# StephenTaf/Modern-Search-Engines-Project

Measured on AMD Instinct MI355X. Metric: queries/sec, two-stage retrieval top-100 (BM25 top-1000 + dense full scan + rerank/fuse), higher is better.
Workload: dtype f32 (exact f32 cosines of every returned document; candidates filtered by one pass of f16 products with a measured margin; batches <= 64 queries: f16x2-split products, |err| <= 8e-6) (dense cosine) / f64 (BM25, fuse)

## Files before the change

### modern-search-engines-project_amd/csrc/msr_gemm.hip

```cpp
#include <type_traits>

#include "msr_common.h"
#include "msr_internal.h"
#include "msr_frag.h"
#include "msr_gemm_dev.h"

namespace {


__global__ __launch_bounds__(256) void unit_bf16_rows_kernel(const float* __restrict__ src, const float* __restrict__ inv_norm,
                                                              int64_t n_rows, int64_t n_pad, bf16x8* __restrict__ dst,
                                                              uint32_t* __restrict__ err_max) {
    const int lane = threadIdx.x & 63;
    const int64_t wave = (int64_t)blockIdx.x * 4 + (threadIdx.x >> 6), n_waves = (int64_t)gridDim.x * 4;
    float worst = 0.f;
    for (int64_t r = wave; r < n_pad; r += n_waves) {
        float ss = 0.f;
#pragma unroll
        for (int h = 0; h < 2; ++h) {
            const int c = lane + 64 * h;
            if (c >= MSR_DIM / 8) continue;
            bf16x8 v;
            if (r < n_rows) {
                const float sc = inv_norm ? inv_norm[r] : 1.0f;
// ... 89 lines not shown
        }
    }
}

__global__ __launch_bounds__(1024) void gemm_kth_kernel(const float* __restrict__ tmax, int n, int stride, int nq, int k,
                                                         const float* __restrict__ margin, float* __restrict__ thr,
                                                         int32_t* __restrict__ flag, float short_val, float margin_scale,
                                                         int raise) {
    __shared__ uint32_t hist[2048];
    __shared__ uint32_t wsum[16];
    __shared__ uint32_t s_bin, s_kk, s_hit;
    const int q = blockIdx.x, t = threadIdx.x, lane = t & 63, wave = t >> 6;
    if (q >= nq) {
        if (t == 0 && !raise) { thr[q] = short_val; if (flag) flag[q] = 0; }
        return;
    }
    const float* row = tmax + (size_t)q * stride;
    uint32_t prefix = 0, mask = 0, kk = (uint32_t)k;
    bool short_row = false;
#pragma unroll 1
    for (int pass = 0; pass < 3; ++pass) {
        const int shift = pass == 0 ? 21 : pass == 1 ? 10 : 0;
        const uint32_t nb = pass == 2 ? 1024u : 2048u;
        hist[t] = 0; hist[t + 1024] = 0;
        if (t == 0) s_hit = 0;
        __syncthreads();
        for (int i = t; i < n; i += 1024) {
            const float x = row[i];
            if (!msr_valid(x)) continue;
            const uint32_t key = msr_ord32(x);
            if ((key & mask) == prefix) atomicAdd(&hist[(key >> shift) & (nb - 1)], 1u);
        }
        __syncthreads();
        const uint32_t h0 = 2 * t < (int)nb ? hist[2 * t] : 0u, h1 = 2 * t + 1 < (int)nb ? hist[2 * t + 1] : 0u;
        const uint32_t c2 = h0 + h1;
        uint32_t inc = c2;
#pragma unroll
        for (int o = 1; o < 64; o <<= 1) {
            const uint32_t v = __shfl_down(inc, o);
            if (lane + o < 64) inc += v;
        }
        if (lane == 0) wsum[wave] = inc;
        __syncthreads();
        uint32_t above = inc - c2;
        for (int w2 = wave + 1; w2 < 16; ++w2) above += wsum[w2];
        if (above < kk && kk <= above + c2) {
            if (above + h1 >= kk) { s_bin = 2 * t + 1; s_kk = kk - above; }
            else { s_bin = 2 * t; s_kk = kk - above - h1; }
            s_hit = 1;
        }
        __syncthreads();
        if (!s_hit) { short_row = true; break; }
        prefix |= s_bin << shift;
        mask |= (nb - 1) << shift;
        kk = s_kk;
        __syncthreads();
    }
    if (t == 0) {
        const float v = short_row ? short_val : msr_unord32(prefix) - (margin ? margin_scale * margin[q] : 0.0f);
        if (raise) {
            if (!short_row && v > thr[q]) thr[q] = v;
        } else {
            thr[q] = v;
            if (flag) flag[q] = short_row ? 1 : 0;
        }
    }
}


__global__ __launch_bounds__(256) void gemm_bucket_kernel(const int4* __restrict__ wgbuf, int wg_cap,
                                                           const int32_t* __restrict__ wg_count,
                                                           const float* __restrict__ thr2, int2* __restrict__ pairs,
                                                           int pair_cap, int32_t* __restrict__ pair_n) {
    const int wg = blockIdx.y;
    int n = wg_count[wg];
    if (n > wg_cap) n = wg_cap;
    for (int i = blockIdx.x * 256 + threadIdx.x; i < n; i += gridDim.x * 256) {
        const int4 e = wgbuf[(size_t)wg * wg_cap + i];
        if (__int_as_float(e.z) >= thr2[e.y]) {
            const int pos = atomicAdd(&pair_n[e.y], 1);
            if (pos < pair_cap) pairs[(size_t)e.y * pair_cap + pos] = make_int2(e.x, e.z);
        }
    }
}

constexpr int GM_PAIR_CAP = 4096;
static_assert(GM_PAIR_CAP <= (1 << 13), "cand_first_len packs first and len into 13 bits each");
__global__ __launch_bounds__(1024) void gemm_cand_kernel(int2* __restrict__ pairs, int32_t* __restrict__ pair_n,
                                                          const int32_t* __restrict__ chunk_doc, int64_t n_rows,
                                                          const int32_t* __restrict__ wg_count, int n_wg, int wg_cap,
                                                          const int32_t* __restrict__ flag, int k,
                                                          const float* __restrict__ margin,
                                                          int32_t* __restrict__ cand_doc, int32_t* __restrict__ cand_first_len,
                                                          int32_t* __restrict__ cand_n) {
    __shared__ uint64_t key[GM_PAIR_CAP];
    __shared__ uint32_t pay[GM_PAIR_CAP];
    __shared__ int s_heads, s_over;
    const int q = blockIdx.x, t = threadIdx.x;
    const int raw = pair_n[q];
    int over = raw > GM_PAIR_CAP || (flag && flag[q]);
    for (int i = t; i < n_wg; i += 1024) over |= wg_count[i] > wg_cap;
    if (t == 0) s_heads = 0;
    s_over = 0;
    __syncthreads();
    if (over) s_over = 1;
    __syncthreads();
    if (s_over) {
        if (t == 0) { cand_n[q] = MSR_SEL_CAP + 1; pair_n[q] = 0; }
        return;
    }
    int P = 64;
    while (P < raw) P <<= 1;
    auto sort_desc = [&]() {
        for (int kk = 2; kk <= P; kk <<= 1)
            for (int j = kk >> 1; j > 0; j >>= 1) {
                for (int idx = t; idx < (P >> 1); idx += 1024) {
                    const int i = ((idx & ~(j - 1)) << 1) | (idx & (j - 1));
                    const int p = i | j;
                    const bool desc = (i & kk) == 0;
                    const uint64_t x = key[i], y = key[p];
                    if (desc ? x < y : x > y) {
                        key[i] = y; key[p] = x;
                        const uint32_t v = pay[i]; pay[i] = pay[p]; pay[p] = v;
                    }
                }
                __syncthreads();
            }
    };
    for (int i = t; i < P; i += 1024) {
        uint64_t kk = 0;
        uint32_t row = 0;
        if (i < raw) {
            const int2 e = pairs[(size_t)q * GM_PAIR_CAP + i];
            if (e.x >= 0 && e.x < n_rows) {
                kk = ((uint64_t)(uint32_t)(chunk_doc[e.x] + 1) << 32) | msr_ord32(__int_as_float(e.y));
                row = (uint32_t)e.x;
            }
        }
        key[i] = kk; pay[i] = row;
    }
    __syncthreads();
    sort_desc();
    uint64_t mine[GM_PAIR_CAP / 1024];
    uint32_t mine_run[GM_PAIR_CAP / 1024];
#pragma unroll
    for (int u = 0; u < GM_PAIR_CAP / 1024; ++u) {
        const int i = t + u * 1024;
        uint64_t kk = 0;
        uint32_t run = 0;
        if (i < P && key[i] != 0) {
            pairs[(size_t)q * GM_PAIR_CAP + i].x = (int32_t)pay[i];
            const uint32_t d = (uint32_t)(key[i] >> 32);
            if (i == 0 || (uint32_t)(key[i - 1] >> 32) != d) {
                kk = ((uint64_t)(uint32_t)key[i] << 32) | (uint32_t)~(uint32_t)(d - 1);
                int len = 1;
                while (i + len < P && (uint32_t)(key[i + len] >> 32) == d) ++len;
                run = (uint32_t)i | ((uint32_t)len << 13);
            }
        }
        mine[u] = kk; mine_run[u] = run;
    }
    __syncthreads();
#pragma unroll
    for (int u = 0; u < GM_PAIR_CAP / 1024; ++u) {
        const int i = t + u * 1024;
        if (i < P) {
            key[i] = mine[u]; pay[i] = mine_run[u];
            if (mine[u]) atomicAdd(&s_heads, 1);
        }
    }
    __syncthreads();
    sort_desc();
    const int heads = s_heads;
    const float tk = heads >= k ? msr_unord32((uint32_t)(key[k - 1] >> 32)) : -__builtin_inff();
    const float cut = tk - margin[q];
    __shared__ int s_keep;
    if (t == 0) s_keep = 0;
    __syncthreads();
    for (int i = t; i < heads; i += 1024)
        if (msr_unord32((uint32_t)(key[i] >> 32)) >= cut) {
            atomicAdd(&s_keep, 1);
            if (i < MSR_SEL_CAP) {
                cand_doc[(size_t)q * MSR_SEL_CAP + i] = (int32_t)~(uint32_t)key[i];
                cand_first_len[(size_t)q * MSR_SEL_CAP + i] = (int32_t)pay[i];
            }
        }
    __syncthreads();
    if (t == 0) { cand_n[q] = s_keep; pair_n[q] = 0; }
}

int g_gemm_dbg = 0;

}

hipError_t msr_unit_bf16_rows(const float* src, const float* inv_norm, int64_t n_rows, int64_t n_pad, void* dst,
                              uint32_t* err_max, hipStream_t stream) {
    if (n_pad <= 0) return hipSuccess;
    hipError_t err = err_max ? hipMemsetAsync(err_max, 0, 4, stream) : hipSuccess;
    if (err != hipSuccess) return err;
    unit_bf16_rows_kernel<<<8192, 256, 0, stream>>>(src, inv_norm, n_rows, n_pad, (bf16x8*)dst, err_max);
    return hipGetLastError();
}

hipError_t msr_batch_margin(const float* qn, int nq, const uint32_t* err_max, float* margin, hipStream_t stream) {
    if (nq <= 0) return hipSuccess;
    batch_margin_kernel<<<(nq + 3) / 4, 256, 0, stream>>>(qn, nq, err_max, margin);
    return hipGetLastError();
}

int msr_gemm_pair_cap() { return GM_PAIR_CAP; }

hipError_t msr_gemm_tmax(const float* tmax_t, int n_j, int parts, int nq_pad, float* out, int out_stride, hipStream_t stream) {
    if (n_j <= 0 || nq_pad <= 0) return hipSuccess;
    if (parts <= 0 || nq_pad % 128 != 0) return hipErrorInvalidValue;
    const dim3 grid((n_j + 31) / 32, nq_pad / 128);
    if (parts == 8) gemm_tmax_kernel<8><<<grid, 256, 0, stream>>>(tmax_t, n_j, parts, nq_pad, out, out_stride);
    else if (parts == 1) gemm_tmax_kernel<1><<<grid, 256, 0, stream>>>(tmax_t, n_j, parts, nq_pad, out, out_stride);
    else gemm_tmax_kernel<0><<<grid, 256, 0, stream>>>(tmax_t, n_j, parts, nq_pad, out, out_stride);
    return hipGetLastError();
}
hipError_t msr_gemm_kth(const float* tmax, int n, int stride, int nq, int nq_pad, int k, const float* margin, float* thr,
                        int32_t* flag, hipStream_t stream, float short_val, float margin_scale, bool raise) {
    if (nq_pad <= 0) return hipSuccess;
    gemm_kth_kernel<<<nq_pad, 1024, 0, stream>>>(tmax, n, stride, nq, k, margin, thr, raise ? nullptr : flag, short_val, margin_scale,
                                                 raise ? 1 : 0);
    return hipGetLastError();
}
hipError_t msr_gemm_bucket(const void* wvbuf, int wv_cap, const int32_t* wv_count, int n_waves, const float* thr2,
                           void* pairs, int32_t* pair_n, hipStream_t stream) {
    gemm_bucket_kernel<<<dim3(2, (unsigned)n_waves), 256, 0, stream>>>((const int4*)wvbuf, wv_cap, wv_count, thr2, (int2*)pairs,
                                                                      GM_PAIR_CAP, pair_n);
    return hipGetLastError();
}
void msr_gemm_set_dbg(int v) { g_gemm_dbg = v; }

hipError_t msr_gemm_candidates(const GemmIndex& g, const DenseIndex& ix, const float* qn, int nq, int k, const float* margin,
                               int32_t* cand_doc, int32_t* cand_first_len, int32_t* cand_n, hipEvent_t* ev, hipStream_t stream) {
    const int nq_pad = (nq + 255) / 256 * 256;
    const int nt = nq_pad / 256;
    if (nq <= 0 || nq_pad > g.max_queries || k < 1 || g.n_tiles < 2 * k) return hipErrorInvalidValue;
    const int grid = g.n_cus / 8 * 8;
    if (grid < 8 || grid / 8 < nt) return hipErrorInvalidValue;
    hipError_t err;
    int ss = g.n_tiles / (8 * k);
    ss = ss < 1 ? 1 : (ss > 16 ? 16 : ss);
#ifdef MSR_DIAG
    if (g_gemm_dbg & 256) ss = 1;
#endif
    const int n_s = (g.n_tiles - ss / 2 + ss - 1) / ss;
    {
        if ((err = msr_stream256_bf16_qimage(qn, nq, nt, g.qmat, stream)) != hipSuccess) return err;
        StreamArgs a{};
        a.E = (const char*)g.emb_n; a.inv_pad = nullptr; a.qimg = (const char*)g.qmat; a.tile_row = g.tile_row;
        a.n_rows = ix.n_chunks; a.tmax_t = g.tmax_t; a.nt = nt; a.q_base = 0; a.append = 0;
        a.t_first = ss / 2; a.t_stride = ss; a.t_count = n_s;
        if (ev && (err = hipEventRecord(ev[0], stream)) != hipSuccess) return err;
        if ((err = msr_stream256_bf16_launch(false, a, grid, stream)) != hipSuccess) return err;
        if (ev && (err = hipEventRecord(ev[1], stream)) != hipSuccess) return err;
        if ((err = msr_gemm_tmax(g.tmax_t, n_s, 1, nq_pad, (float*)g.tmax, g.tmax_stride, stream)) != hipSuccess) return err;
        gemm_kth_kernel<<<nq_pad, 1024, 0, stream>>>((const float*)g.tmax, n_s, g.tmax_stride, nq, k, margin, g.thr, g.flag, __builtin_inff(), 1.0f, 0);
        a.t_first = 0; a.t_stride = 1; a.t_count = g.n_tiles;
        a.thr = g.thr; a.wvbuf = g.wgbuf; a.wv_cap = g.wv_cap; a.wv_count = g.wv_count;
        if (ev && (err = hipEventRecord(ev[2], stream)) != hipSuccess) return err;
        if ((err = msr_stream256_bf16_launch(true, a, grid, stream)) != hipSuccess) return err;
        if (ev && (err = hipEventRecord(ev[3], stream)) != hipSuccess) return err;
        if ((err = msr_gemm_tmax(g.tmax_t, g.n_tiles, 1, nq_pad, (float*)g.tmax, g.tmax_stride, stream)) != hipSuccess) return err;
        gemm_kth_kernel<<<nq_pad, 1024, 0, stream>>>((const float*)g.tmax, g.n_tiles, g.tmax_stride, nq, k, margin, g.thr2, nullptr, __builtin_inff(), 1.0f, 0);
    }
    gemm_bucket_kernel<<<dim3(2, (unsigned)grid * 8), 256, 0, stream>>>((const int4*)g.wgbuf, g.wv_cap, g.wv_count, g.thr2,
                                                                       (int2*)g.pairs, GM_PAIR_CAP, g.pair_n);
    gemm_cand_kernel<<<nq, 1024, 0, stream>>>((int2*)g.pairs, g.pair_n, ix.chunk_doc, ix.n_chunks, g.wv_count, grid * 8, g.wv_cap,
                                              g.flag, k, margin, cand_doc, cand_first_len, cand_n);
    return hipGetLastError();
}
```

### modern-search-engines-project_amd/csrc/msr_gemm_f32.hip

```cpp
#include <cmath>
#include <type_traits>

#include "msr_common.h"
#include "msr_internal.h"
#include "msr_frag.h"
#include "msr_gemm_dev.h"

namespace {

constexpr int GF_THREADS = 512;
constexpr int GF_KT = MSR_DIM / 32;
constexpr int GF_ROWB = MSR_DIM * 4;
constexpr int GF_PAIR_CAP = 4096;

typedef StreamArgs GemmF32Args;

__device__ __forceinline__ const char* uniform_ptr(const char* p) {
    const uint64_t u = (uint64_t)p;
    const uint32_t lo = __builtin_amdgcn_readfirstlane((uint32_t)u), hi = __builtin_amdgcn_readfirstlane((uint32_t)(u >> 32));
    return (const char*)(((uint64_t)hi << 32) | lo);
}

constexpr int GS_NB = 8;
constexpr int GS_STEP = 8192;
// ... 248 lines not shown
template <int OFF, bool NT = false>
__device__ __forceinline__ void gload16s(f32x4& r, uint32_t voff, uint64_t sbase) {
    if (NT) asm volatile("global_load_dwordx4 %0, %1, %2 offset:%3 nt" : "=v"(r) : "v"(voff), "s"(sbase), "n"(OFF) : "memory");
    else asm volatile("global_load_dwordx4 %0, %1, %2 offset:%3" : "=v"(r) : "v"(voff), "s"(sbase), "n"(OFF) : "memory");
}
__device__ __forceinline__ f16x8 take16(const f32x4& r) {
    f32x4 o;
    asm volatile("v_mov_b32 %0, %1" : "=v"(o[0]) : "v"(r[0]));
    asm volatile("v_mov_b32 %0, %1" : "=v"(o[1]) : "v"(r[1]));
    asm volatile("v_mov_b32 %0, %1" : "=v"(o[2]) : "v"(r[2]));
    asm volatile("v_mov_b32 %0, %1" : "=v"(o[3]) : "v"(r[3]));
    return __builtin_bit_cast(f16x8, o);
}
__device__ __forceinline__ uint32_t fresh_lane() {
    uint32_t l;
    asm volatile("v_mbcnt_lo_u32_b32 %0, -1, 0\n\tv_mbcnt_hi_u32_b32 %0, -1, %0" : "=v"(l));
    return l;
}
typedef __attribute__((address_space(3))) char lds_char;
template <int OFF>
__device__ __forceinline__ void lds_read16(f16x8& r, uint32_t addr) {
    asm volatile("ds_read_b128 %0, %1 offset:%2" : "=v"(r) : "v"(addr), "n"(OFF) : "memory");
}
__device__ __forceinline__ uint64_t uniform_u64(uint64_t u) {
    const uint32_t lo = __builtin_amdgcn_readfirstlane((uint32_t)u), hi = __builtin_amdgcn_readfirstlane((uint32_t)(u >> 32));
    return ((uint64_t)hi << 32) | lo;
}

template <bool EMIT, bool BF16, bool TILED = false, bool NTL = false, bool F16I = false>
__global__ __launch_bounds__(G2_THREADS) void gemm_stream256_kernel(GemmF32Args a) {
    static_assert(!F16I || (BF16 && !TILED && !NTL), "the f16 image takes the 16-bit image's data path");
    static_assert(!(BF16 && TILED), "the fragment-order copy exists for the f32 rows only");
    extern __shared__ __attribute__((aligned(16))) char smem[];
    constexpr int ROWB = BF16 ? MSR_DIM * 2 : GF_ROWB;
    constexpr int KPS = BF16 ? 2 : 1;
    constexpr int RSLOTS = G2_NB / KPS;
    constexpr int NMI = 2, NNI = 16;
    constexpr int WROWS = 16 * NMI;
    static_assert((G2_THREADS / 64) * WROWS == MSR_STREAM256_TILE_ROWS, "the fragment-order copy is padded for this many rows per tile visit");
    const int tid = threadIdx.x, lane = tid & 63;
    const int w = __builtin_amdgcn_readfirstlane(tid >> 6);
    const int wr = w, wc = 0;
    const int li16 = lane & 15, lg = lane >> 4;
    const int nt = a.nt;
    int G = (int)gridDim.x, gid = (int)blockIdx.x, grp = 0;
    bool active = true;
    if (nt > 1) {
        const int per_x = (int)gridDim.x >> 3, xcd = (int)blockIdx.x & 7, li = (int)blockIdx.x >> 3;
        const int gpx = per_x / nt, mg = li / nt;
        grp = li - mg * nt;
        G = __builtin_amdgcn_readfirstlane(8 * gpx);
        gid = __builtin_amdgcn_readfirstlane(xcd * gpx + mg);
        grp = __builtin_amdgcn_readfirstlane(grp);
        active = mg < gpx;
    }
    const int nq_pad = nt * 256;
    int wave_cnt = EMIT && a.append ? __builtin_amdgcn_readfirstlane(a.wv_count[blockIdx.x * 8 + w]) : 0;
    int4* wvbuf = EMIT ? (int4*)a.wvbuf + ((size_t)blockIdx.x * 8 + w) * a.wv_cap : nullptr;
    if (!active || gid >= a.t_count) {
        if (EMIT && lane == 0) a.wv_count[blockIdx.x * 8 + w] = wave_cnt;
        return;
    }
    const int n_mine = __builtin_amdgcn_readfirstlane((a.t_count - gid + G - 1) / G);
    const char* qimg = a.qimg + (size_t)grp * (GF_KT * G2_STEP);
    const int q_base = a.q_base + grp * 256;
    float* thr_lds = (float*)(smem + 2 * G2_BLK);
    if (EMIT && tid < 256) thr_lds[tid] = a.thr[grp * 256 + tid];
    constexpr bool THR_REGS = EMIT && !BF16;
    uint32_t thr_h[THR_REGS ? NNI / 2 : 1];
    if (THR_REGS) {
        auto down_h = [](float x) -> uint32_t {
            _Float16 h = (_Float16)x;
            uint16_t b = __builtin_bit_cast(uint16_t, h);
            if ((float)h > x) b = (b & 0x8000u) ? (uint16_t)(b + 1) : (b == 0 ? (uint16_t)0x8001u : (uint16_t)(b - 1));
            return b;
        };
#pragma unroll
        for (int j = 0; j < NNI / 2; ++j) {
            const float lo = a.thr[grp * 256 + (2 * j) * 16 + li16], hi = a.thr[grp * 256 + (2 * j + 1) * 16 + li16];
            thr_h[j] = down_h(lo) | (down_h(hi) << 16);
        }
    }
    constexpr bool JOIN = BF16;
    uint32_t* tmx = (uint32_t*)(smem + G2_TMX);
    if (JOIN) tmx[tid] = 0u;
    auto flush_tmax = [&](int tile_j, int par) {
        const int ln = (int)fresh_lane();
        if (ln < 32) {
            uint32_t* slot = tmx + par * 256 + w * 32 + ln;
            a.tmax_t[(size_t)tile_j * nq_pad + grp * 256 + w * 32 + ln] = ord_val(*slot);
            *slot = 0u;
        }
    };
    float* inv_lds = (float*)(smem + 2 * G2_BLK + 1024) + w * 64;
    auto stage_b = [&](int blk, int pb) {
        const char* base = uniform_ptr(qimg + (size_t)blk * G2_BLK + (size_t)w * 8192);
#pragma unroll
        for (int i = 0; i < 8; ++i)
            __builtin_amdgcn_global_load_lds((glb_void*)(base + (uint32_t)(i * 1024 + lane * 16)),
                                             (lds_void*)(smem + pb * G2_BLK + w * 8192 + i * 1024), 16, 0, 0);
    };
    f32x4 acc[NMI][NNI];
#pragma unroll
    for (int mi = 0; mi < NMI; ++mi)
#pragma unroll
        for (int ni = 0; ni < NNI; ++ni) acc[mi][ni] = (f32x4){0.f, 0.f, 0.f, 0.f};

    auto tile_of = [&](int j) { return a.t_first + j * a.t_stride; };
    auto tile_base = [&](int row0) { return uniform_u64((uint64_t)a.E + (uint64_t)row0 * ROWB); };
    constexpr int NV = (BF16 || TILED) ? 1 : NMI;
    auto row_off = [&](int row0, int mi) -> uint32_t {
        if (TILED) return (uint32_t)(lane * 16);
        if (BF16) return (uint32_t)((WROWS * wr + li16) * ROWB + lg * 32);
        int64_t r = (int64_t)row0 + WROWS * wr + 16 * mi + li16;
        if (r > a.n_rows - 1) r = a.n_rows - 1;
        return (uint32_t)((r - row0) * ROWB + lg * 32);
    };
    int jt = gid;
    int row0 = a.tile_row[tile_of(jt)], row_end = a.tile_row[tile_of(jt) + 1];
    int jn = jt + G < a.t_count ? jt + G : jt;
    int row0n = a.tile_row[tile_of(jn)];
    uint64_t bp = tile_base(TILED ? a.tile_trow[tile_of(jt)] : row0), bn = tile_base(TILED ? a.tile_trow[tile_of(jn)] : row0n);
    uint32_t vp[NV], vn[NV];
#pragma unroll
    for (int mi = 0; mi < NV; ++mi) { vp[mi] = row_off(row0, mi); vn[mi] = row_off(row0n, mi); }

    static_assert(NMI == 2, "the wait counts below assume 4 row loads per ring slot");
    f32x4 ring[RSLOTS][NMI][2];
    auto load_rows = [&](auto slot_c, uint64_t sb, const uint32_t* v, auto off_c) {
        constexpr int slot = decltype(slot_c)::value, off = decltype(off_c)::value;
#pragma unroll
        for (int mi = 0; mi < NMI; ++mi) {
            if (TILED) {
                const uint64_t b = sb + (uint64_t)((2 * wr + mi) * ((GF_KT / KPS) * 2048) + slot * 2048);
                gload16s<0, NTL>(ring[slot][mi][0], v[0], b);
                gload16s<1024, NTL>(ring[slot][mi][1], v[0], b);
            } else {
                const uint64_t b = BF16 ? sb + (uint64_t)(mi * 16 * ROWB) : sb;
                gload16s<off, NTL>(ring[slot][mi][0], v[BF16 ? 0 : mi], b);
                gload16s<off + 16, NTL>(ring[slot][mi][1], v[BF16 ? 0 : mi], b);
            }
        }
    };
    auto pin_rows = [&](auto slot_c) {
        constexpr int slot = decltype(slot_c)::value;
        pin4(ring[slot][0][0], ring[slot][0][1], ring[slot][1][0], ring[slot][1][1]);
    };
    constexpr int NKB = GF_KT / G2_NB;
    constexpr int BLKB = TILED ? RSLOTS * 2048 : RSLOTS * 128;
    stage_b(0, 0);
#pragma unroll
    for (int s = 0; s < RSLOTS; ++s)
#pragma unroll
        for (int mi = 0; mi < NMI; ++mi) ring[s][mi][0] = ring[s][mi][1] = (f32x4){0.f, 0.f, 0.f, 0.f};
    load_rows(std::integral_constant<int, 0>{}, bp, vp, std::integral_constant<int, 0>{});
    load_rows(std::integral_constant<int, 1>{}, bp, vp, std::integral_constant<int, 128>{});
    if (!BF16) {
        load_rows(std::integral_constant<int, RSLOTS - 2>{}, bp, vp, std::integral_constant<int, 256>{});
        load_rows(std::integral_constant<int, RSLOTS - 1>{}, bp, vp, std::integral_constant<int, 384>{});
    }
    wait_vm0();
    pin_rows(std::integral_constant<int, 0>{}); pin_rows(std::integral_constant<int, 1>{});
    pin_rows(std::integral_constant<int, RSLOTS - 2>{}); pin_rows(std::integral_constant<int, RSLOTS - 1>{});
    wg_barrier();
    int pb = 0;

// ... 101 lines not shown
        for (int kb = 0; kb < NKB; ++kb) {
            const bool last = kb == NKB - 1;
            const int kn = last ? 0 : kb + 1;
#ifdef MSR_DIAG
            if (!(a.dbg & 524288))
#endif
            stage_b(kn, pb ^ 1);
            step(std::integral_constant<int, 0>{}, kn, last);
            step(std::integral_constant<int, 1>{}, kn, last);
            step(std::integral_constant<int, 2>{}, kn, last);
            step(std::integral_constant<int, 3>{}, kn, last);
            if (BF16) asm volatile("s_waitcnt vmcnt(8)" ::: "memory");
            else asm volatile("s_waitcnt vmcnt(16)" ::: "memory");
#ifdef MSR_DIAG
            if (!(a.dbg & 131072))
#endif
            wg_barrier();
            pb ^= 1;
            if (JOIN && kb == 0 && it > 0) flush_tmax(jt_prev, (it - 1) & 1);
        }
        const int ln_e = (int)fresh_lane();
        const int lg_e = ln_e >> 4;
        f32x4 inv4[NMI];
        if (!BF16 || F16I) {
            if (F16I) asm volatile("s_waitcnt vmcnt(8)" ::: "memory");
            else asm volatile("s_waitcnt vmcnt(12)" ::: "memory");
#pragma unroll
            for (int mi = 0; mi < NMI; ++mi) inv4[mi] = *(const f32x4*)(inv_lds + mi * 16 + 4 * lg_e);
        }
        const int n_valid = row_end - row0;
        const int col_e = wc * 128 + (ln_e & 15);
        float thr_nx = (EMIT && !THR_REGS) ? thr_lds[col_e] : 0.f;
#ifdef MSR_DIAG
        if (a.dbg & 65536) {
#pragma unroll
            for (int ni = 0; ni < NNI; ++ni)
#pragma unroll
                for (int mi = 0; mi < NMI; ++mi) acc[mi][ni] = (f32x4){0.f, 0.f, 0.f, 0.f};
        } else
#endif
#pragma unroll
        for (int ni = 0; ni < NNI; ++ni) {
            f32x4 v[NMI];
            float cmax = NEG_INF;
            const float thr_cur = thr_nx;
            if (EMIT && !THR_REGS && ni + 1 < NNI) thr_nx = thr_lds[(ni + 1) * 16 + col_e];
#pragma unroll
            for (int mi = 0; mi < NMI; ++mi) {
                const int blk = wr * WROWS + mi * 16;
                if (BF16 && !F16I) v[mi] = acc[mi][ni];
                else v[mi] = acc[mi][ni] * inv4[mi];
                if (blk + 16 > n_valid) {
#pragma unroll
                    for (int rr = 0; rr < 4; ++rr)
                        if (blk + 4 * lg_e + rr >= n_valid) v[mi][rr] = NEG_INF;
                }
                cmax = max2_raw(cmax, max3_raw(max2_raw(v[mi][0], v[mi][1]), v[mi][2], v[mi][3]));
                acc[mi][ni] = (f32x4){0.f, 0.f, 0.f, 0.f};
            }
            if (EMIT) {
                float thr;
                if (THR_REGS) thr = (float)__builtin_bit_cast(_Float16, (uint16_t)(ni & 1 ? thr_h[ni >> 1] >> 16 : thr_h[ni >> 1] & 0xffffu));
                else thr = thr_cur;
                if (__ballot(cmax >= thr) != 0) {
                    const int q = q_base + ni * 16 + col_e;
#pragma unroll
                    for (int mi = 0; mi < NMI; ++mi) {
                        const int rb = wr * WROWS + mi * 16 + 4 * lg_e;
#pragma unroll
                        for (int rr = 0; rr < 4; ++rr) {
                            const float x = v[mi][rr];
                            const bool hit = x >= thr;
                            const unsigned long long hm = __ballot(hit);
                            if (hm != 0) {
                                const int pos = wave_cnt + (int)__builtin_amdgcn_mbcnt_hi((uint32_t)(hm >> 32), __builtin_amdgcn_mbcnt_lo((uint32_t)hm, 0u));
                                if (hit && pos < a.wv_cap)
                                    wvbuf[pos] = make_int4(row0 + rb + rr, q, __float_as_int(x), tile_of(jt));
                                wave_cnt += __popcll(hm);
                            }
                        }
                    }
                }
            }
            float m = cmax;
            auto s32 = __builtin_amdgcn_permlane32_swap(__float_as_uint(m), __float_as_uint(m), false, false);
            m = max2_raw(__uint_as_float(s32[0]), __uint_as_float(s32[1]));
            auto s16 = __builtin_amdgcn_permlane16_swap(__float_as_uint(m), __float_as_uint(m), false, false);
            m = max2_raw(__uint_as_float(s16[0]), __uint_as_float(s16[1]));
            if (JOIN) {
                if (lg_e == 0) atomicMax(tmx + (it & 1) * 256 + ni * 16 + col_e, ord_key(m));
            } else {
                if (lg_e == 0) a.tmax_t[((size_t)jt * 8 + w) * nq_pad + grp * 256 + ni * 16 + col_e] = m;
            }
        }
        jt_prev = jt;
        jt = jn;
        row0 = row0n;
        row_end = a.tile_row[tile_of(jt) + 1];
        jn = jt + G < a.t_count ? jt + G : jt;
        row0n = a.tile_row[tile_of(jn)];
        bp = bn; bn = tile_base(TILED ? a.tile_trow[tile_of(jn)] : row0n);
#pragma unroll
        for (int mi = 0; mi < NV; ++mi) { vp[mi] = vn[mi]; vn[mi] = row_off(row0n, mi); }
    }
    wait_vm0();
    if (JOIN) {
        wg_barrier();
        flush_tmax(jt_prev, (n_mine - 1) & 1);
    }
    if (EMIT && lane == 0) a.wv_count[blockIdx.x * 8 + w] = wave_cnt;
}

template <bool BF16, bool TOBF16 = BF16>
__global__ __launch_bounds__(256) void build_qimg2_kernel(const float* __restrict__ qn, int nq, f16x8* __restrict__ qimg) {
    const int i = blockIdx.x * 256 + threadIdx.x;
    if (i >= GF_KT * 256 * 4) return;
    const int g = blockIdx.y;
    const int cp = i & 3, ql = (i >> 2) & 255, kt = i >> 10;
    const int q = 256 * g + ql;
    const int c = cp ^ (((ql >> 3) & 1) << 1);
    f16x8 h;
    if (q < nq) {
        const float* src = qn + (size_t)q * MSR_DIM + (BF16 ? 64 * (kt >> 1) + 16 * c + 8 * (kt & 1) : 32 * kt + 8 * c);
        if (TOBF16) {
            bf16x8 b;
#pragma unroll
            for (int j = 0; j < 8; ++j) b[j] = (__bf16)src[j];
            h = __builtin_bit_cast(f16x8, b);
        } else {
            h = cvt_f16_rtn(*(const f32x4*)src, *(const f32x4*)(src + 4));
        }
    } else {
#pragma unroll
        for (int j = 0; j < 8; ++j) h[j] = (_Float16)0.f;
    }
    qimg[(size_t)g * (GF_KT * 256 * 4) + i] = h;
}

__global__ __launch_bounds__(256) void build_qimg1_kernel(const float* __restrict__ qn, int nq, f16x8* __restrict__ qimg) {
    const int i = blockIdx.x * 256 + threadIdx.x;
    if (i >= GF_KT * 128 * 4) return;
    const int g = blockIdx.y;
    const int cp = i & 3, ql = (i >> 2) & 127, kt = i >> 9;
    const int q = 128 * g + ql;
    const int c = cp ^ (((ql >> 3) & 1) << 1);
    f16x8 h;
    if (q < nq) {
        const float* src = qn + (size_t)q * MSR_DIM + 32 * kt + 8 * c;
        h = cvt_f16_rtn(*(const f32x4*)src, *(const f32x4*)(src + 4));
    } else {
#pragma unroll
        for (int j = 0; j < 8; ++j) h[j] = (_Float16)0.f;
    }
    qimg[(size_t)g * (GF_KT * 128 * 4) + i] = h;
}

__global__ __launch_bounds__(256) void pad_inv_kernel(const float* __restrict__ inv, int64_t n, int64_t n_pad, float* __restrict__ out) {
    const int64_t i = (int64_t)blockIdx.x * 256 + threadIdx.x;
    if (i < n_pad) out[i] = i < n ? inv[i] : 1.0f;
}

__global__ __launch_bounds__(256) void f16_row_error_kernel(const float* __restrict__ src, const float* __restrict__ inv_norm,
                                                             int64_t n_rows, uint32_t* __restrict__ err_max) {
    const int lane = threadIdx.x & 63;
    const int64_t wave = (int64_t)blockIdx.x * 4 + (threadIdx.x >> 6), n_waves = (int64_t)gridDim.x * 4;
    float worst = 0.f;
    for (int64_t r = wave; r < n_rows; r += n_waves) {
        const f32x4* p = (const f32x4*)(src + (size_t)r * MSR_DIM);
        float ss = 0.f;
#pragma unroll
        for (int h = 0; h < 3; ++h) {
            const f32x4 x = p[lane + 64 * h];
            ss += f16_err2(x.x) + f16_err2(x.y) + f16_err2(x.z) + f16_err2(x.w);
        }
        for (int o = 32; o > 0; o >>= 1) ss += __shfl_xor(ss, o);
// ... 214 lines not shown
    if ((dbg & 16777216) && grid >= 2 * k && p.n_s > grid) {
        p.n_s = p.n_s / grid * grid;
        p.ss = T / p.n_s;
    }
#endif
    const double root = std::sqrt((double)T * (double)p.n_s);
    int want3 = 0;
#ifdef MSR_DIAG
    want3 = dbg & 2097152;
#endif
    if (want3) {
        const double r = std::cbrt((double)T / (double)p.n_s);
        const int m1 = (int)std::floor(p.n_s * r / grid + 0.5), m2 = (int)std::floor(p.n_s * r * r / grid + 0.5);
        const int64_t t1 = (int64_t)m1 * grid, t2 = (int64_t)m2 * grid;
        if (m1 >= 1 && m2 > m1 && t1 >= 2 * k && T - t2 >= grid) {
            p.n_seg = 3; p.bound[1] = (int)t1; p.bound[2] = (int)t2; p.bound[3] = T;
            return p;
        }
    }
    int64_t t1 = (int64_t)std::floor(root / grid + 0.5) * grid;
#ifdef MSR_DIAG
    if (dbg & 4194304) t1 = std::max<int64_t>(grid, t1 / 2 / grid * grid);
    if (dbg & 8388608) t1 = 2 * t1;
#endif
    if (t1 >= std::max(grid, 2 * k) && T - t1 >= grid) {
        p.n_seg = 2; p.bound[1] = (int)t1; p.bound[2] = T;
    }
    return p;
}

}

hipError_t msr_gemm_f32_pass(const GemmF32Index& g, const DenseIndex& ix, const float* qn, int nq, int k, int k_part,
                             float* out_part, hipEvent_t* ev, int* width_out, int* seg_out, hipStream_t stream) {
    const int W = nq > 128 ? 256 : 128;
    const int waves = 8;
    const int G = (nq + W - 1) / W;
    if (nq <= 0 || G * W > 128 * g.max_groups || k < 1 || g.n_tiles < 2 * k) return hipErrorInvalidValue;
    if (width_out) *width_out = W;
    hipError_t err;
    int NT0 = 1;
    if (W == 256 && (g.n_cus & 7) == 0) NT0 = std::min(std::min(G, g.max_nt), g.n_cus >> 3);
    bool image16 = W == 256 && NT0 > 1 && g.emb_f16 != nullptr;
#ifdef MSR_DIAG
    if (g_f32_dbg & (2048 | 1048576)) image16 = false;
#endif
    if (image16) build_qimg2_kernel<true, false><<<dim3((GF_KT * 256 * 4 + 255) / 256, G), 256, 0, stream>>>(qn, nq, (f16x8*)g.qimg);
    else if (W == 256) build_qimg2_kernel<false><<<dim3((GF_KT * 256 * 4 + 255) / 256, G), 256, 0, stream>>>(qn, nq, (f16x8*)g.qimg);
    else build_qimg1_kernel<<<dim3((GF_KT * 128 * 4 + 255) / 256, G), 256, 0, stream>>>(qn, nq, (f16x8*)g.qimg);
    f16_margin_kernel<<<(nq + 3) / 4, 256, 0, stream>>>(qn, nq, g.err_max, g.margin);
    const float* margin = g.margin;
    const int grid = g.n_cus;
    const PassShape shape = pass_shape(g.n_tiles, k, grid, g.single_emit != 0, g_f32_dbg);
    const int ss = shape.ss, n_s = shape.n_s;
    if (seg_out) *seg_out = shape.n_seg;
    const size_t qimg_bytes = (size_t)GF_KT * W * 64;
    int NT = 1;
    if (W == 256 && (grid & 7) == 0) NT = std::min(std::min(G, g.max_nt), grid >> 3);
#ifdef MSR_DIAG
    if (g_f32_dbg & 2048) NT = 1;
    if (g_f32_dbg & 4096) NT = std::min(NT, 2);
#endif
    GemmF32Args a{};
    a.dbg = g_f32_dbg; a.nt = 1;
    a.E = (const char*)ix.emb; a.inv_pad = g.inv_pad; a.tile_row = g.tile_row;
    bool tiled = W == 256 && g.emb_tiled != nullptr && !image16;
#ifdef MSR_DIAG
    if (g_f32_dbg & 8192) tiled = false;
#endif
    if (tiled) { a.E = (const char*)g.emb_tiled; a.tile_trow = g.tile_trow; }
    if (image16) a.E = (const char*)g.emb_f16;
    const int tmax_parts = image16 ? 1 : waves;
    a.n_rows = ix.n_chunks; a.tmax_t = g.tmax_t;
    a.t_first = ss / 2; a.t_stride = ss; a.t_count = n_s;
    for (int gi = 0; gi < G; gi += NT) {
        a.nt = std::min(NT, G - gi);
        a.qimg = (const char*)g.qimg + gi * qimg_bytes;
        if (ev && gi == 0 && (err = hipEventRecord(ev[0], stream)) != hipSuccess) return err;
        if ((err = launch_f32(W, false, a, grid, stream, tiled, image16)) != hipSuccess) return err;
        if (ev && gi == 0 && (err = hipEventRecord(ev[1], stream)) != hipSuccess) return err;
        if ((err = msr_gemm_tmax(g.tmax_t, n_s, tmax_parts, W * a.nt, g.tmax + (size_t)gi * W * g.tmax_stride, g.tmax_stride, stream)) != hipSuccess) return err;
    }
    if ((err = msr_gemm_kth(g.tmax, n_s, g.tmax_stride, nq, W * G, k, margin, g.thr, g.flag, stream)) != hipSuccess) return err;
    a.t_stride = 1;
    a.wvbuf = g.wvbuf; a.wv_cap = g.wv_cap * (8 / waves); a.wv_count = g.wv_count;
    for (int s = 0; s < shape.n_seg; ++s) {
        const int t0 = shape.bound[s], t1 = shape.bound[s + 1];
        a.t_first = t0; a.t_count = t1 - t0;
        for (int gi = 0; gi < G; gi += NT) {
            a.nt = std::min(NT, G - gi);
            a.qimg = (const char*)g.qimg + gi * qimg_bytes;
            a.thr = g.thr + gi * W; a.q_base = gi * W; a.append = (s > 0 || gi > 0);
            if (ev && gi == 0 && s == 0 && (err = hipEventRecord(ev[2], stream)) != hipSuccess) return err;
            if ((err = launch_f32(W, true, a, grid, stream, tiled, image16)) != hipSuccess) return err;
            if (ev && gi == 0 && s == shape.n_seg - 1 && (err = hipEventRecord(ev[3], stream)) != hipSuccess) return err;
            if ((err = msr_gemm_tmax(g.tmax_t, t1 - t0, tmax_parts, W * a.nt, g.tmax + (size_t)gi * W * g.tmax_stride + t0, g.tmax_stride, stream)) != hipSuccess) return err;
        }
        if (s + 1 < shape.n_seg &&
            (err = msr_gemm_kth(g.tmax, t1, g.tmax_stride, nq, W * G, k, margin, g.thr, nullptr, stream, __builtin_inff(), 1.0f, true)) != hipSuccess)
            return err;
    }
    if ((err = msr_gemm_kth(g.tmax, g.n_tiles, g.tmax_stride, nq, W * G, k, margin, g.thr2, nullptr, stream)) != hipSuccess) return err;
    if (out_part && (err = msr_gemm_kth(g.tmax, g.n_tiles, g.tmax_stride, nq, nq, k_part, margin, out_part, nullptr, stream,
                                        -__builtin_inff(), 0.5f)) != hipSuccess) return err;
    return hipSuccess;
}

namespace {
__global__ __launch_bounds__(256) void raise_thr_kernel(float* __restrict__ thr2, const float* __restrict__ bound,
                                                         const float* __restrict__ margin, int nq) {
    const int q = blockIdx.x * 256 + threadIdx.x;
    if (q >= nq) return;
    const float b = bound[q] - 0.5f * margin[q];
    if (b > thr2[q]) thr2[q] = b;
}
}

hipError_t msr_gemm_f32_finish(const GemmF32Index& g, const DenseIndex& ix, const float* qn, int nq, int k, const float* bound,
                               int32_t* out_doc, float* out_score, int32_t* out_chunk, int32_t* out_n, int32_t* gate,
                               hipStream_t stream) {
    const int waves = 8, grid = g.n_cus;
    const int wv_cap = g.wv_cap * (8 / waves);
    if (nq <= 0 || k < 1) return hipErrorInvalidValue;
    hipError_t err;
    if (bound) {
        raise_thr_kernel<<<(nq + 255) / 256, 256, 0, stream>>>(g.thr2, bound, g.margin, nq);
        if ((err = hipGetLastError()) != hipSuccess) return err;
    }
    if ((err = msr_gemm_bucket(g.wvbuf, wv_cap, g.wv_count, grid * waves, g.thr2, g.pairs, g.pair_n, stream)) != hipSuccess) return err;
    gemm_f32_cand_kernel<<<nq, 1024, 0, stream>>>((int2*)g.pairs, g.pair_n, ix.chunk_doc, ix.n_chunks, g.wv_count, grid * waves,
                                                  wv_cap, g.flag, g.cand_doc, g.cand_chunk, g.cand_n, gate);
    if ((err = hipGetLastError()) != hipSuccess) return err;
    return msr_batch_rescore_rows(ix, qn, nq, k, (const int32_t*)g.pairs, 2, GF_PAIR_CAP, g.cand_doc, g.cand_score, g.cand_chunk,
                                  g.cand_n, out_doc, out_score, out_chunk, out_n, stream);
}

hipError_t msr_gemm_f32_topk(const GemmF32Index& g, const DenseIndex& ix, const float* qn, int nq, int k,
                             int32_t* out_doc, float* out_score, int32_t* out_chunk,
                             int32_t* out_n, int32_t* gate, hipEvent_t* ev, int* width_out, int* seg_out, hipStream_t stream) {
    hipError_t err = msr_gemm_f32_pass(g, ix, qn, nq, k, k, nullptr, ev, width_out, seg_out, stream);
    if (err != hipSuccess) return err;
    return msr_gemm_f32_finish(g, ix, qn, nq, k, nullptr, out_doc, out_score, out_chunk, out_n, gate, stream);
}
```

### modern-search-engines-project_amd/csrc/msr_internal.h

```cpp
#pragma once
#include <hip/hip_runtime.h>
#include <stdint.h>

#define MSR_DIM 768
#define MSR_SEL_BINS 4096
#define MSR_SEL_CAP 4096

struct SelState {
    uint64_t pref_hi, mask_hi;
    uint32_t pref_lo, mask_lo;
    int32_t k_rem;
    int32_t n_above;
    int32_t done;
    int32_t n_sel;
};

struct SelScratch {
    uint32_t* hist;
    SelState* state;
    uint64_t* cand_hi;
    uint32_t* cand_lo;
    int32_t* cand_n;
    const int32_t* gate;
    int gate_per64;
// ... 189 lines not shown
hipError_t msr_prep_queries(const float* q, int nq, float* qn, int nq_pad, hipStream_t stream);
hipError_t msr_fill_chunk_doc(const int32_t* doc_off, int64_t n_docs, int32_t* chunk_doc, hipStream_t stream);
hipError_t msr_row_inv_norm(const float* emb, int64_t n_rows, float* inv_norm, hipStream_t stream);
hipError_t msr_interleave(const float* src, int64_t n_rows, float* dst, hipStream_t stream);
hipError_t msr_best_chunk(const DenseIndex& ix, const float* qn, int nq, int k, int max_chunks,
                          const int32_t* out_doc, const int32_t* out_n, int32_t* out_chunk, hipStream_t stream);

hipError_t msr_check_range(const int32_t* v, int64_t n, int64_t hi, int32_t* flag, hipStream_t stream);
hipError_t msr_gather_rows_run(const DenseIndex& ix, const int32_t* rows, int n, float* out, hipStream_t stream);
hipError_t msr_group_row_sets(const int32_t* group_off, int n_groups, const int32_t* g_set, int32_t* row_set, hipStream_t stream);
struct GroupedMergeArgs {
    const int32_t* l_doc; const float* l_score; const int32_t* l_chunk; const int32_t* l_n;
    int32_t kk;
    const int32_t* group_off;
    const int32_t* excl_off;
    const int32_t* excl_doc;
    int32_t k;
    float min_score;
    int32_t* out_doc; float* out_score; int32_t* out_chunk; int32_t* out_src; int32_t* out_n;
    uint64_t* g_hi; uint32_t* g_lo; uint32_t* g_val;
};
hipError_t msr_grouped_merge(const GroupedMergeArgs& a, int n_groups, hipStream_t stream);

struct RerankParams {
    double smoothing, max_boost, max_decay;
    int32_t max_chunks;
};
#define MSR_RERANK_RECORD_WORDS 16
struct RerankRecords {
    int32_t* out;
    const int32_t* q_base;
    const int32_t* blk_off;
    int64_t capacity;
    int q_first;
};
hipError_t msr_rerank_gather(const DenseIndex& ix, const int32_t* url_group, const float* qn, int nq,
                             const int32_t* cand_doc, const int32_t* cand_n, int max_cand, int doc_base,
                             int row_base, int max_chunks, float* cos_out ,
                             int32_t* meta , int q_per_block, int64_t block_stride,
                             const RerankRecords& rec, hipStream_t stream);
hipError_t msr_rerank_plan_run(int nq, const int32_t* cand_doc, const int32_t* cand_n, int max_cand, const int32_t* bounds,
                               int n_shards, int my, int qps, int32_t* counts, int32_t* send_base, int32_t* blk_off,
                               int32_t* recv_off, int32_t* pair, hipStream_t stream);
hipError_t msr_rerank_scatter_run(const int32_t* records, int64_t capacity, const int32_t* counts, const int32_t* recv_off, int n_shards, int nq,
                                  int qps, int q_first, int n_mine, int max_cand, float* cos_out, int32_t* meta_out,
                                  hipStream_t stream);
hipError_t msr_rerank_fuse_run(int nq, const int32_t* cand_doc, const double* cand_bm25, const int32_t* cand_n,
                               int max_cand, const RerankParams& p, const float* cos_in, const int32_t* meta,
                               int32_t* out_doc, double* out_score, double* out_orig, int32_t* out_chunk,
                               int32_t* out_n, int32_t* out_rows, hipStream_t stream);

hipError_t msr_diversify_run(int nq, const int32_t* f_doc, const double* f_score, const double* f_orig, const int32_t* f_chunk,
                             const int32_t* f_n, int max_cand, const int32_t* doc_domain, int64_t n_domain_docs, int top_k,
                             double threshold, int diversify, int32_t* out_doc, double* out_score, double* out_orig,
                             int32_t* out_chunk, int32_t* out_n, hipStream_t stream);

hipError_t msr_or_parts(const void* in, int n_parts, int64_t part_stride_bytes, int64_t n_words, void* out, hipStream_t stream);

struct GemmIndex {
    const void* emb_n;
    const int32_t* tile_row;
    int32_t n_tiles;
    int32_t n_cus;
    int32_t max_queries;
    void* qmat;
    float* tmax;
    int32_t tmax_stride;
    float* tmax_t;
    float* thr; float* thr2;
    int32_t* flag;
    void* wgbuf;
    int32_t wv_cap;
    int32_t* wv_count;
    void* pairs;
    int32_t* pair_n;
};
int msr_gemm_pair_cap();
hipError_t msr_gemm_tmax(const float* tmax_t, int n_j, int parts, int nq_pad, float* out, int out_stride, hipStream_t stream);
hipError_t msr_gemm_kth(const float* tmax, int n, int stride, int nq, int nq_pad, int k, const float* margin, float* thr,
                        int32_t* flag, hipStream_t stream, float short_val = __builtin_inff(), float margin_scale = 1.0f,
                        bool raise = false);
hipError_t msr_gemm_bucket(const void* wvbuf, int wv_cap, const int32_t* wv_count, int n_waves, const float* thr2,
                           void* pairs, int32_t* pair_n, hipStream_t stream);
void msr_bm25_set_dbg(int v);
void msr_gemm_set_dbg(int v);
hipError_t msr_unit_bf16_rows(const float* src, const float* inv_norm, int64_t n_rows, int64_t n_pad, void* dst,
                              uint32_t* err_max, hipStream_t stream);
hipError_t msr_batch_margin(const float* qn, int nq, const uint32_t* err_max, float* margin, hipStream_t stream);
hipError_t msr_gemm_candidates(const GemmIndex& g, const DenseIndex& ix, const float* qn, int nq, int k, const float* margin,
                               int32_t* cand_doc, int32_t* cand_first_len, int32_t* cand_n, hipEvent_t* ev,
                               hipStream_t stream);

constexpr int MSR_STREAM256_TILE_ROWS = 256;

struct StreamArgs {
    const char* E;
    const float* inv_pad;
    const char* qimg;
    const int32_t* tile_row;
    const int32_t* tile_trow;
    int64_t n_rows;
    int t_first, t_stride, t_count;
    float* tmax_t;
    const float* thr;
    void* wvbuf; int wv_cap; int32_t* wv_count;
    int q_base;
    int append;
    int nt;
    int dbg;
};
hipError_t msr_stream256_bf16_launch(bool emit, const StreamArgs& a, int grid, hipStream_t stream);
hipError_t msr_stream256_bf16_qimage(const float* qn, int nq, int n_groups, void* qimg, hipStream_t stream);

struct GemmF32Index {
    const int32_t* tile_row;
    int32_t n_tiles;
    int32_t n_cus;
    int32_t max_groups;
    const float* inv_pad;
    void* qimg;
    float* tmax_t;
    float* tmax;
    int32_t tmax_stride;
    float* thr; float* thr2; int32_t* flag;
    void* wvbuf; int32_t wv_cap; int32_t* wv_count;
    void* pairs; int32_t* pair_n;
    uint32_t* err_max; float* margin;
    int32_t* cand_doc; float* cand_score; int32_t* cand_chunk; int32_t* cand_n;
    int32_t max_nt;
    const void* emb_tiled;
    const int32_t* tile_trow;
    const void* emb_f16;
    int32_t single_emit;
};
hipError_t msr_f16_rows(const float* emb, int64_t n_rows, int64_t n_pad, void* out, hipStream_t stream);
hipError_t msr_tile_rows(const float* emb, const int32_t* tile_row, const int32_t* tile_trow, int n_tiles, void* emb_tiled,
                         hipStream_t stream);
hipError_t msr_f16_row_error(const float* emb, const float* inv_norm, int64_t n_rows, uint32_t* err_max, hipStream_t stream);
void msr_gemm_f32_set_dbg(int v);
hipError_t msr_pad_inv_norm(const float* inv, int64_t n, int64_t n_pad, float* out, hipStream_t stream);
hipError_t msr_gemm_f32_topk(const GemmF32Index& g, const DenseIndex& ix, const float* qn, int nq, int k,
                             int32_t* out_doc, float* out_score, int32_t* out_chunk,
                             int32_t* out_n, int32_t* gate, hipEvent_t* ev, int* width_out, int* seg_out, hipStream_t stream);
hipError_t msr_gemm_f32_pass(const GemmF32Index& g, const DenseIndex& ix, const float* qn, int nq, int k, int k_part,
                             float* out_part, hipEvent_t* ev, int* width_out, int* seg_out, hipStream_t stream);
hipError_t msr_gemm_f32_finish(const GemmF32Index& g, const DenseIndex& ix, const float* qn, int nq, int k, const float* bound,
                               int32_t* out_doc, float* out_score, int32_t* out_chunk, int32_t* out_n, int32_t* gate,
                               hipStream_t stream);

hipError_t msr_batch_rescore_rows(const DenseIndex& ix, const float* qn, int nq, int k, const int32_t* rows, int row_stride,
                                  int row_cap, int32_t* cand_doc, float* cand_score, int32_t* cand_chunk, int32_t* cand_n,
                                  int32_t* out_doc, float* out_score, int32_t* out_chunk, int32_t* out_n, hipStream_t stream);
hipError_t msr_batch_finish(const DenseIndex& ix, const float* qn, int nq, int k, int max_chunks, const float* margin,
                            const float* scores, const float* top_score, const int32_t* top_n, int32_t* cand_doc,
                            float* cand_score, int32_t* cand_chunk, int32_t* cand_n, int32_t* out_doc,
                            float* out_score, int32_t* out_chunk, int32_t* out_n, hipStream_t stream);
```

Before: 61460.

## Derive per-tile maxima from emitted entries instead of in-kernel tmax reduction

For the f32 emit pass with W==256 and no f16 image, the GEMM kernel skips its per-tile max reduction (permlane swaps plus tmax_t stores). The tmax table is instead filled with -inf and rebuilt after each segment from the emitted candidate entries using integer atomic max/min. This removes the tmax_t traffic and the separate tmax reduction launch, at the cost of a clear kernel and an atomic scatter kernel per segment. Because the maxima now cover only emitted entries, the threshold raising between segments may be looser.

```diff
diff --git a/modern-search-engines-project_amd/csrc/msr_gemm.hip b/modern-search-engines-project_amd/csrc/msr_gemm.hip
--- a/modern-search-engines-project_amd/csrc/msr_gemm.hip
+++ b/modern-search-engines-project_amd/csrc/msr_gemm.hip
@@ -195,6 +195,26 @@
             if (pos < pair_cap) pairs[(size_t)e.y * pair_cap + pos] = make_int2(e.x, e.z);
         }
     }
+}
+
+__global__ __launch_bounds__(256) void gemm_entry_tmax_kernel(const int4* __restrict__ wgbuf, int wg_cap,
+                                                               const int32_t* __restrict__ wg_count,
+                                                               float* __restrict__ tmax, int stride, int tile_lo, int n_tiles,
+                                                               int nq_pad) {
+    const int wg = blockIdx.x;
+    int n = wg_count[wg];
+    if (n > wg_cap) n = wg_cap;
+    for (int i = threadIdx.x; i < n; i += 256) {
+        const int4 e = wgbuf[(size_t)wg * wg_cap + i];
+        if ((unsigned)e.y >= (unsigned)nq_pad || e.w < tile_lo || e.w >= n_tiles) continue;
+        float* p = tmax + (size_t)e.y * stride + e.w;
+        if (e.z >= 0) atomicMax((int*)p, e.z);
+        else atomicMin((unsigned int*)p, (unsigned int)e.z);
+    }
+}
+__global__ __launch_bounds__(256) void gemm_fill_kernel(f32x4* __restrict__ dst, size_t n4, float v) {
+    const size_t i = (size_t)blockIdx.x * 256 + threadIdx.x;
+    if (i < n4) dst[i] = (f32x4){v, v, v, v};
 }
 
 constexpr int GM_PAIR_CAP = 4096;
@@ -343,6 +363,20 @@
                            void* pairs, int32_t* pair_n, hipStream_t stream) {
     gemm_bucket_kernel<<<dim3(2, (unsigned)n_waves), 256, 0, stream>>>((const int4*)wvbuf, wv_cap, wv_count, thr2, (int2*)pairs,
                                                                       GM_PAIR_CAP, pair_n);
+    return hipGetLastError();
+}
+hipError_t msr_gemm_tmax_clear(float* tmax, int stride, int nq_pad, hipStream_t stream) {
+    const size_t n4 = (size_t)nq_pad * stride / 4;
+    if (n4 == 0) return hipSuccess;
+    if (stride % 4 != 0) return hipErrorInvalidValue;
+    gemm_fill_kernel<<<(unsigned)((n4 + 255) / 256), 256, 0, stream>>>((f32x4*)tmax, n4, -__builtin_inff());
+    return hipGetLastError();
+}
+hipError_t msr_gemm_entry_tmax(const void* wvbuf, int wv_cap, const int32_t* wv_count, int n_waves, float* tmax, int stride,
+                               int tile_lo, int n_tiles, int nq_pad, hipStream_t stream) {
+    if (tile_lo < 0 || n_tiles > stride) return hipErrorInvalidValue;
+    gemm_entry_tmax_kernel<<<(unsigned)n_waves, 256, 0, stream>>>((const int4*)wvbuf, wv_cap, wv_count, tmax, stride, tile_lo,
+                                                                 n_tiles, nq_pad);
     return hipGetLastError();
 }
 void msr_gemm_set_dbg(int v) { g_gemm_dbg = v; }
diff --git a/modern-search-engines-project_amd/csrc/msr_gemm_f32.hip b/modern-search-engines-project_amd/csrc/msr_gemm_f32.hip
--- a/modern-search-engines-project_amd/csrc/msr_gemm_f32.hip
+++ b/modern-search-engines-project_amd/csrc/msr_gemm_f32.hip
@@ -354,6 +354,11 @@
         }
     }
     constexpr bool JOIN = BF16;
+#ifdef MSR_DIAG
+    const bool TMAX = !EMIT || JOIN || (a.dbg & 33554432);
+#else
+    constexpr bool TMAX = !EMIT || JOIN;
+#endif
     uint32_t* tmx = (uint32_t*)(smem + G2_TMX);
     if (JOIN) tmx[tid] = 0u;
     auto flush_tmax = [&](int tile_j, int par) {
@@ -621,15 +626,17 @@
                     }
                 }
             }
-            float m = cmax;
-            auto s32 = __builtin_amdgcn_permlane32_swap(__float_as_uint(m), __float_as_uint(m), false, false);
-            m = max2_raw(__uint_as_float(s32[0]), __uint_as_float(s32[1]));
-            auto s16 = __builtin_amdgcn_permlane16_swap(__float_as_uint(m), __float_as_uint(m), false, false);
-            m = max2_raw(__uint_as_float(s16[0]), __uint_as_float(s16[1]));
-            if (JOIN) {
-                if (lg_e == 0) atomicMax(tmx + (it & 1) * 256 + ni * 16 + col_e, ord_key(m));
-            } else {
-                if (lg_e == 0) a.tmax_t[((size_t)jt * 8 + w) * nq_pad + grp * 256 + ni * 16 + col_e] = m;
+            if (TMAX) {
+                float m = cmax;
+                auto s32 = __builtin_amdgcn_permlane32_swap(__float_as_uint(m), __float_as_uint(m), false, false);
+                m = max2_raw(__uint_as_float(s32[0]), __uint_as_float(s32[1]));
+                auto s16 = __builtin_amdgcn_permlane16_swap(__float_as_uint(m), __float_as_uint(m), false, false);
+                m = max2_raw(__uint_as_float(s16[0]), __uint_as_float(s16[1]));
+                if (JOIN) {
+                    if (lg_e == 0) atomicMax(tmx + (it & 1) * 256 + ni * 16 + col_e, ord_key(m));
+                } else {
+                    if (lg_e == 0) a.tmax_t[((size_t)jt * 8 + w) * nq_pad + grp * 256 + ni * 16 + col_e] = m;
+                }
             }
         }
         jt_prev = jt;
@@ -1010,6 +1017,11 @@
         if ((err = msr_gemm_tmax(g.tmax_t, n_s, tmax_parts, W * a.nt, g.tmax + (size_t)gi * W * g.tmax_stride, g.tmax_stride, stream)) != hipSuccess) return err;
     }
     if ((err = msr_gemm_kth(g.tmax, n_s, g.tmax_stride, nq, W * G, k, margin, g.thr, g.flag, stream)) != hipSuccess) return err;
+    bool entry_tmax = W == 256 && !image16;
+#ifdef MSR_DIAG
+    if (g_f32_dbg & 33554432) entry_tmax = false;
+#endif
+    if (entry_tmax && (err = msr_gemm_tmax_clear(g.tmax, g.tmax_stride, W * G, stream)) != hipSuccess) return err;
     a.t_stride = 1;
     a.wvbuf = g.wvbuf; a.wv_cap = g.wv_cap * (8 / waves); a.wv_count = g.wv_count;
     for (int s = 0; s < shape.n_seg; ++s) {
@@ -1022,8 +1034,11 @@
             if (ev && gi == 0 && s == 0 && (err = hipEventRecord(ev[2], stream)) != hipSuccess) return err;
             if ((err = launch_f32(W, true, a, grid, stream, tiled, image16)) != hipSuccess) return err;
             if (ev && gi == 0 && s == shape.n_seg - 1 && (err = hipEventRecord(ev[3], stream)) != hipSuccess) return err;
-            if ((err = msr_gemm_tmax(g.tmax_t, t1 - t0, tmax_parts, W * a.nt, g.tmax + (size_t)gi * W * g.tmax_stride + t0, g.tmax_stride, stream)) != hipSuccess) return err;
-        }
+            if (!entry_tmax &&
+                (err = msr_gemm_tmax(g.tmax_t, t1 - t0, tmax_parts, W * a.nt, g.tmax + (size_t)gi * W * g.tmax_stride + t0, g.tmax_stride, stream)) != hipSuccess) return err;
+        }
+        if (entry_tmax && (err = msr_gemm_entry_tmax(g.wvbuf, a.wv_cap, g.wv_count, grid * waves, g.tmax, g.tmax_stride, t0,
+                                                     g.n_tiles, W * G, stream)) != hipSuccess) return err;
         if (s + 1 < shape.n_seg &&
             (err = msr_gemm_kth(g.tmax, t1, g.tmax_stride, nq, W * G, k, margin, g.thr, nullptr, stream, __builtin_inff(), 1.0f, true)) != hipSuccess)
             return err;
diff --git a/modern-search-engines-project_amd/csrc/msr_internal.h b/modern-search-engines-project_amd/csrc/msr_internal.h
--- a/modern-search-engines-project_amd/csrc/msr_internal.h
+++ b/modern-search-engines-project_amd/csrc/msr_internal.h
@@ -295,6 +295,9 @@
                         bool raise = false);
 hipError_t msr_gemm_bucket(const void* wvbuf, int wv_cap, const int32_t* wv_count, int n_waves, const float* thr2,
                            void* pairs, int32_t* pair_n, hipStream_t stream);
+hipError_t msr_gemm_tmax_clear(float* tmax, int stride, int nq_pad, hipStream_t stream);
+hipError_t msr_gemm_entry_tmax(const void* wvbuf, int wv_cap, const int32_t* wv_count, int n_waves, float* tmax, int stride,
+                               int tile_lo, int n_tiles, int nq_pad, hipStream_t stream);
 void msr_bm25_set_dbg(int v);
 void msr_gemm_set_dbg(int v);
 hipError_t msr_unit_bf16_rows(const float* src, const float* inv_norm, int64_t n_rows, int64_t n_pad, void* dst,
```

Result: faster. 63990, median of 6 (+4.1%).
